# ssheybani/baby-vision-curriculum

Hardware: AMD Instinct MI355X
Metric: video clips/sec (node) VideoMAE-base 16x224^2 bf16 pretraining (higher is better)
Workload: dtype bf16; 1 GPU; VideoMAE-base (ViT-B/16 encoder, 4-layer decoder), 16x224x224 clips, tubelet 2, 90% tube mask, full training step (fwd + MSE + bwd + GradScaler + SGD-Nesterov); clips_per_gpu=256, global_batch=256, parallelism=dp1, weights=random init N(0,0.02), seed 0

## Files before the change

__graft_entry__.py:

```python
import importlib.util
import os
import subprocess
import sys

ROOT = os.path.dirname(os.path.abspath(__file__))
PKG_DIR = os.path.join(ROOT, "baby-vision-curriculum_amd")
CSRC = os.path.join(PKG_DIR, "csrc")
LIB = os.path.join(PKG_DIR, "libbvc_hip.so")
PRODUCT_SOURCES = ["gemm.hip", "gemm_persist.hip", "gemm8.hip", "gemm_as.hip", "attention.hip", "attention_probs.hip", "retrieval.hip", "separability.hip", "rowops.hip", "optim_layerwise.hip", "stack.hip", "context.hip", "ops.hip", "augment.hip", "randaug.hip", "jpeg.hip", "videomae.hip", "jepa.hip", "comm.hip"]
EXPERIMENT_SOURCES = [os.path.join("experiments", "gemm_big.hip"), os.path.join("experiments", "gemm_pp.hip")]
EXPERIMENT_INCLUDES = [os.path.join("experiments", "attention_dq_wave96.inc")]
HEADERS = ["common.h", "dropgate.h", "augment.h", "randaug.h", "jpeg.h", "gemm.h", "gemm_tile.h", "gemm_kernel_body.inc", "attention.h", "attention_fwd_body.inc", "attention_dq_body.inc", "attention_dkdv_body.inc", "rowops.h", "optim_layerwise.h", "stack.h", "context.h", os.path.join("..", "..", "include", "bvc.h")]


def _experiments():
    return "BVC_EXPERIMENTS" in os.environ.get("BVC_EXTRA_HIPCC_FLAGS", "")


def _sources():
    return PRODUCT_SOURCES + (EXPERIMENT_SOURCES if _experiments() else [])


SOURCES = PRODUCT_SOURCES


EXPERIMENT_FLAGS = {"attention.hip": ["-mllvm", "-amdgpu-mfma-vgpr-form=1"]}


def _extra_flags(src):
    return EXPERIMENT_FLAGS.get(src, []) if _experiments() else []


HASH_FILE = LIB + ".srchash"


def _source_hash():
    import hashlib
    h = hashlib.sha256()
    for f in _sources() + HEADERS + (EXPERIMENT_INCLUDES if _experiments() else []):
        with open(os.path.join(CSRC, f), "rb") as fh:
            h.update(f.encode() + b"\0" + fh.read())
    h.update(os.environ.get("BVC_EXTRA_HIPCC_FLAGS", "").encode())
    return h.hexdigest()


def _stale():
    if not (os.path.exists(LIB) and os.path.exists(HASH_FILE)):
        return True
    with open(HASH_FILE) as fh:
        return fh.read().strip() != _source_hash()


def _hash_of(files):
    import hashlib
    h = hashlib.sha256()
    for f in files:
        with open(os.path.join(CSRC, f), "rb") as fh:
            h.update(f.encode() + b"\0" + fh.read())
    return h.hexdigest()


def build(force: bool = False) -> None:
    if force or _stale():
        from concurrent.futures import ThreadPoolExecutor
        hipcc = os.environ.get("HIPCC", "/opt/rocm/bin/hipcc")
        objdir = os.path.join(PKG_DIR, "build")
        os.makedirs(objdir, exist_ok=True)
        flags = ["--offload-arch=gfx950", "-O3", "-std=c++17", "-fPIC"] + os.environ.get("BVC_EXTRA_HIPCC_FLAGS", "").split()

        def compile_one(src):
            obj = os.path.join(objdir, os.path.basename(src).replace(".hip", ".o"))
            stamp = obj + ".hash"
            fl = flags + _extra_flags(src) + ["-I" + CSRC]
            want = _hash_of([src] + HEADERS + (EXPERIMENT_INCLUDES if _experiments() else [])) + " " + " ".join(fl)
            if not force and os.path.exists(obj) and os.path.exists(stamp) and open(stamp).read() == want:
                return obj
            cmd = [hipcc, *fl, "-c", os.path.join(CSRC, src), "-o", obj]
            if src == "gemm8.hip":
                r = subprocess.run(cmd + ["-Rpass-analysis=kernel-resource-usage"], stderr=subprocess.PIPE, text=True)
                if r.returncode != 0:
                    sys.stderr.write(r.stderr)
                    raise subprocess.CalledProcessError(r.returncode, cmd)
                name = None
                for line in r.stderr.splitlines():
                    if "Function Name:" in line:
                        name = line.split("Function Name:")[1].split()[0]
                    elif "VGPRs Spill:" in line and name and "gemm8_kernel" in name and name.endswith("ELi0EEEvNS_9GemmGroupEi"):
                        if int(line.split("VGPRs Spill:")[1].split()[0]) != 0:
                            raise RuntimeError(f"gemm8.hip: {name} spills VGPRs; its counted-wait epilogue assumes none")
            else:
                subprocess.run(cmd, check=True)
            with open(stamp, "w") as fh:
# ... 59 lines not shown
```

baby-vision-curriculum_amd/csrc/gemm.h:

```cpp
#pragma once
#include "common.h"
#include "dropgate.h"
#include "../../include/bvc.h"

namespace bvc {

enum GemmLayout { GEMM_NT = BVC_GEMM_NT, GEMM_NN = BVC_GEMM_NN, GEMM_TN = BVC_GEMM_TN };

enum GemmEpilogue {
    EPI_F32 = BVC_EPI_F32,
    EPI_BF16 = BVC_EPI_BF16,
    EPI_GELU = BVC_EPI_GELU,
    EPI_RESID = BVC_EPI_RESID,
    EPI_POS = BVC_EPI_POS,
    EPI_E2D = BVC_EPI_E2D,
    EPI_LOSS = BVC_EPI_LOSS,
    EPI_DGELU = BVC_EPI_DGELU,
    EPI_F32_BF16 = BVC_EPI_F32_BF16,
    EPI_RELU = BVC_EPI_RELU,
    EPI_DRELU = BVC_EPI_DRELU,
    EPI_NCE = BVC_EPI_NCE,
    EPI_NCE_BWD = BVC_EPI_NCE_BWD,
    EPI_RESID_LN = BVC_EPI_RESID_LN,
    EPI_DLN = BVC_EPI_DLN,
    EPI_RESID_GATE = BVC_EPI_RESID_GATE
};

using GemmProblem = bvc_gemm_desc;

constexpr int kMaxGroup = 4;

struct Options { int gemm8 = 0; int dw_overlap = 0; int row_ln = 0; int row_stagger = 1; int deterministic = 0; int head_pad = 0; int dec_tail = 1; int dec_first = -1; };
Options& options();

float* det_scratch(size_t floats, hipStream_t stream);
size_t det_scratch_bytes();
int det_scratch_release();

struct DryRun { bool on = false; char name[160] = ""; };
DryRun& dry_run();

constexpr size_t operand_tail_bytes(size_t bf16_columns) { return 64 * bf16_columns * 2 + 1024; }
constexpr bool tn_tail_ok(int K, int ld) { return K % 64 == 0 || ((size_t)K + 63) / 64 * 64 * (size_t)ld * 2 + 1024 <= 0x100000000ull; }

int launch_gemm(const GemmProblem* probs, int nprob, GemmLayout layout, int tile_cfg, hipStream_t stream, int stages = -1);

int launch_gemm_gate(const GemmProblem& p, const Gate& gate, int tile_cfg, hipStream_t stream);

int gemm_num_tiles(const GemmProblem& p, int tile_cfg);
int gemm_pick_tile(const GemmProblem* probs, int nprob, int tile_cfg);
bool gemm_row_ln_ok(int M, int N, int K);
constexpr size_t kRowLnPartFloats = 512 * 2 * 384;

}
```

baby-vision-curriculum_amd/csrc/gemm.hip:

```cpp
#include <stdio.h>
#include <stdlib.h>
#include <string.h>

#include <algorithm>
#include <mutex>
#include <vector>

#include "gemm_tile.h"

namespace bvc {

Options& options() {
    static Options o;
    return o;
}
DryRun& dry_run() {
    static thread_local DryRun d;
    return d;
}

template <int BM, int BN, bool AT, bool BT, int NS, int LB = 2, bool EARLY_ = true>
__global__ __launch_bounds__(256, LB) void gemm_kernel(const GemmGroup g) {
    constexpr bool DET = false;
#include "gemm_kernel_body.inc"
// ... 46 lines not shown

namespace {
struct DetBuf { int dev; hipStream_t stream; float* ptr; size_t floats; };
std::mutex& det_mutex() { static std::mutex m; return m; }
std::vector<DetBuf>& det_bufs() { static std::vector<DetBuf> v; return v; }
}

float* det_scratch(size_t floats, hipStream_t stream) {
    int dev = 0;
    if (hipGetDevice(&dev) != hipSuccess) { set_error("det_scratch: hipGetDevice failed"); return nullptr; }
    std::lock_guard<std::mutex> lock(det_mutex());
    for (DetBuf& b : det_bufs()) {
        if (b.dev != dev || b.stream != stream) continue;
        if (b.floats >= floats) return b.ptr;
        if (hipStreamSynchronize(stream) != hipSuccess || hipFree(b.ptr) != hipSuccess) {
            set_error("det_scratch: releasing the old workspace failed");
            return nullptr;
        }
        const size_t want = std::max(floats, b.floats + b.floats / 2);
        b.ptr = nullptr; b.floats = 0;
        if (hipMalloc(&b.ptr, want * sizeof(float)) != hipSuccess) {
            set_error("det_scratch: hipMalloc of %zu bytes failed", want * sizeof(float));
            b.ptr = nullptr;
            return nullptr;
        }
        b.floats = want;
        return b.ptr;
    }
    DetBuf b{dev, stream, nullptr, floats};
    if (hipMalloc(&b.ptr, floats * sizeof(float)) != hipSuccess) {
        set_error("det_scratch: hipMalloc of %zu bytes failed", floats * sizeof(float));
        return nullptr;
    }
    det_bufs().push_back(b);
    return b.ptr;
}

int det_scratch_release() {
    int dev = 0;
    BVC_CHECK_HIP(hipGetDevice(&dev));
    std::lock_guard<std::mutex> lock(det_mutex());
    BVC_CHECK_HIP(hipDeviceSynchronize());
    std::vector<DetBuf>& v = det_bufs();
    for (size_t i = 0; i < v.size();) {
        if (v[i].dev != dev) { ++i; continue; }
        BVC_CHECK_HIP(hipFree(v[i].ptr));
        v.erase(v.begin() + i);
    }
    return BVC_OK;
}

size_t det_scratch_bytes() {
    int dev = 0;
    if (hipGetDevice(&dev) != hipSuccess) return 0;
    std::lock_guard<std::mutex> lock(det_mutex());
    size_t n = 0;
    for (const DetBuf& b : det_bufs())
        if (b.dev == dev) n += b.floats * sizeof(float);
    return n;
}

static void tile_dims(int cfg, int& bm, int& bn) {
    if (cfg == 10 || cfg == 11) { bm = 256; bn = cfg == 10 ? 256 : 128; return; }
    if (cfg == 12) { bm = 128; bn = 384; return; }
    if (cfg == 14) { bm = 128; bn = 256; return; }
    bm = cfg == 2 ? 64 : 128;
    bn = cfg == 0 ? 128 : 64;
}

static int tiles_for(const GemmProblem& p, int cfg) {
    int bm, bn;
    tile_dims(cfg, bm, bn);
    return ((p.M + bm - 1) / bm) * ((p.N + bn - 1) / bn);
}

bool gemm_row_ln_ok(int M, int N, int K) { return N == 384 && K % 64 == 0 && K >= 128 && M > 0 && (double)M * 1536.0 < 4294000000.0; }

int gemm_pick_tile(const GemmProblem* probs, int nprob, int tile_cfg) {
    if (tile_cfg == 6 || tile_cfg == 7) return tile_cfg - 6;
    if (tile_cfg == 9) return 0;
    if (tile_cfg >= 10 && tile_cfg <= 12) return tile_cfg;
    if (tile_cfg == 14) return tile_cfg;
    if (tile_cfg >= 15 && tile_cfg <= 18) return 0;
    if (tile_cfg >= 0) return tile_cfg;
    int t0 = 0, t1 = 0, nmax = 0;
    for (int i = 0; i < nprob; ++i) {
        t0 += tiles_for(probs[i], 0) * probs[i].split_k;
        t1 += tiles_for(probs[i], 1) * probs[i].split_k;
        nmax = probs[i].N > nmax ? probs[i].N : nmax;
    }
    if (nmax <= 384) return t0 >= 1024 ? 0 : (t1 >= 256 ? 1 : 2);
    if (t0 >= 400) return 0;
    if (t1 >= 400) return 1;
    return 2;
}

static int pick_panel(const GemmProblem& p, int cfg, GemmLayout layout) {
    if (BVC_EXP_ENV("BVC_GEMM_LEGACY_WALK") != nullptr) return 0;
    if (const char* pe = BVC_EXP_ENV("BVC_GEMM_PANEL")) {
        const int tn = (p.N + (cfg == 10 ? 256 : 128) - 1) / (cfg == 10 ? 256 : 128), gq = atoi(pe);
        if (layout != GEMM_TN && gq > 0) return gq < tn ? gq : tn;
    }
    if (layout == GEMM_TN) return 0;
    int bm, bn;
    tile_dims(cfg, bm, bn);
    const int tiles_m = (p.M + bm - 1) / bm, tiles_n = (p.N + bn - 1) / bn;
    const double kper = (double)((p.K + p.split_k - 1) / p.split_k);
    const double a_slab = bm * kper * 2.0, b_slab = bn * kper * 2.0, cap = 2.0 * 1024 * 1024;
    const double rows_x = tiles_m / 8.0 > 1.0 ? tiles_m / 8.0 : 1.0;
    auto cost = [&](int G) {
        const double npan = (double)((tiles_n + G - 1) / G);
        const double waves = rows_x * G / 64.0 > 1.0 ? rows_x * G / 64.0 : 1.0;
        return rows_x * a_slab * npan + tiles_n * b_slab * (G * b_slab <= cap ? 1.0 : waves);
    };
    int gmax = (int)(cap / b_slab);
    if ((cfg == 10 || cfg == 11) && gmax < 2) {
        const int gq = cfg == 10 ? 6 : 8;
        return gq < tiles_n ? gq : tiles_n;
    }
    if (gmax < 1) gmax = 1;
    if (gmax >= tiles_n) return tiles_n;
    const int npan = (tiles_n + gmax - 1) / gmax;
    const int G = (tiles_n + npan - 1) / npan;
    return cost(G) < cost(tiles_n) ? G : tiles_n;
}

static int pick_gemm8(const GemmProblem* probs, int nprob, GemmLayout layout);
int gemm_num_tiles(const GemmProblem& p, int tile_cfg) {
    if (tile_cfg < 0) {
        const int g8 = pick_gemm8(&p, 1, GEMM_NT);
        if (g8 > 0) tile_cfg = g8;
    }
    return tiles_for(p, gemm_pick_tile(&p, 1, tile_cfg));
}

template <int BM, int BN, bool AT, bool BT, int NS, int LB = 2, bool EARLY = true>
static int launch_one(const GemmGroup& g, int nblocks, hipStream_t stream) {
    constexpr size_t lds = (size_t)NS * (BM + BN) * 64 * 2;
    if (dry_run().on) {
        snprintf(dry_run().name, sizeof(dry_run().name), "bvc::gemm_kernel<%d, %d, %s, %s, %d, %d, %s>", BM, BN, AT ? "true" : "false",
                 BT ? "true" : "false", NS, LB, EARLY ? "true" : "false");
        return BVC_OK;
    }
    static bool attr_set = false;
    if (lds > 65536 && !attr_set) {
        BVC_CHECK_HIP(hipFuncSetAttribute(reinterpret_cast<const void*>(&gemm_kernel<BM, BN, AT, BT, NS, LB, EARLY>),
                                          hipFuncAttributeMaxDynamicSharedMemorySize, (int)lds));
        attr_set = true;
    }
    hipLaunchKernelGGL((gemm_kernel<BM, BN, AT, BT, NS, LB, EARLY>), dim3(nblocks), dim3(256), lds, stream, g);
    BVC_CHECK_HIP(hipGetLastError());
    return BVC_OK;
}

template <int BM, int BN, bool AT, bool BT>
static int launch_det_one(const GemmGroup& g, int nblocks, hipStream_t stream) {
    constexpr size_t lds = (size_t)2 * (BM + BN) * 64 * 2;
    static_assert(lds <= 65536, "gemm_det_kernel: dynamic LDS above 64 KiB would need the attribute");
    if (dry_run().on) {
        snprintf(dry_run().name, sizeof(dry_run().name), "bvc::gemm_det_kernel<%d, %d, %s, %s>", BM, BN, AT ? "true" : "false", BT ? "true" : "false");
        return BVC_OK;
    }
    hipLaunchKernelGGL((gemm_det_kernel<BM, BN, AT, BT>), dim3(nblocks), dim3(256), lds, stream, g);
    BVC_CHECK_HIP(hipGetLastError());
    return BVC_OK;
}

template <int BM, int BN>
static int launch_det_cfg(const GemmGroup& g, GemmLayout layout, int nblocks, hipStream_t stream) {
    switch (layout) {
        case GEMM_NT: return launch_det_one<BM, BN, false, false>(g, nblocks, stream);
        case GEMM_NN: return launch_det_one<BM, BN, false, true>(g, nblocks, stream);
        case GEMM_TN: return launch_det_one<BM, BN, true, true>(g, nblocks, stream);
        default: set_error("launch_gemm: bad layout %d", (int)layout); return BVC_ERR_INVALID;
    }
}

template <int BM, int BN, int NS>
static int launch_cfg(const GemmGroup& g, GemmLayout layout, int nblocks, hipStream_t stream) {
    switch (layout) {
        case GEMM_NT: return launch_one<BM, BN, false, false, NS>(g, nblocks, stream);
        case GEMM_NN: return launch_one<BM, BN, false, true, NS>(g, nblocks, stream);
        case GEMM_TN: return launch_one<BM, BN, true, true, NS>(g, nblocks, stream);
        default: set_error("launch_gemm: bad layout %d", (int)layout); return BVC_ERR_INVALID;
    }
}

template <int BM, int BN>
static int launch_stages(const GemmGroup& g, GemmLayout layout, int stages, int nblocks, hipStream_t stream) {
    if (stages == 3 && layout == GEMM_TN) return launch_one<BM, BN, true, true, 2, 1>(g, nblocks, stream);
    if (stages == 4) {
        if (layout == GEMM_NT) return launch_one<BM, BN, false, false, 2, 2, false>(g, nblocks, stream);
        if (layout == GEMM_NN) return launch_one<BM, BN, false, true, 2, 2, false>(g, nblocks, stream);
        return launch_one<BM, BN, true, true, 2, 2, false>(g, nblocks, stream);
    }
    return launch_cfg<BM, BN, 2>(g, layout, nblocks, stream);
}

int gemm_pick_stages(int, GemmLayout, int, int stages) { return (stages == 3 || stages == 4) ? stages : 2; }

int launch_gemm_big_nt(const GemmProblem& p, int cfg, hipStream_t stream);
int launch_gemm_persist(const GemmGroup& g, GemmLayout layout, int cfg, hipStream_t stream, int defer);
int launch_gemm8(const GemmGroup& g, GemmLayout layout, int bn, hipStream_t stream, bool det = false);
int launch_gemm_as(const GemmProblem& p, GemmLayout layout, int variant, hipStream_t stream);
bool gemm_as_ok(const GemmProblem& p, GemmLayout layout);
int launch_gemm_pp(const GemmGroup& g, GemmLayout layout, hipStream_t stream);

static int pick_gemm8(const GemmProblem* probs, int nprob, GemmLayout layout) {
    const int mode = options().gemm8;
    if (mode < 0 || nprob != 1 || layout == GEMM_TN) return -1;
    const GemmProblem& p = probs[0];
    if (p.split_k != 1 || p.K % 64 != 0) return -1;
    if (p.a_bytes >= 0x80000000u || p.b_bytes >= 0x80000000u) return -1;
    const bool gated = p.epi == EPI_DGELU || p.epi == EPI_DRELU;
    const bool bf = p.epi == EPI_BF16 || p.epi == EPI_GELU || p.epi == EPI_RELU;
    const bool resid = (p.epi == EPI_RESID || p.epi == EPI_POS || p.epi == EPI_F32 || p.epi == EPI_LOSS) && layout == GEMM_NT;
    if (!bf && !resid && !gated) return -1;
    const int tm = (p.M + 255) / 256, tn256 = (p.N + 255) / 256, tn128 = (p.N + 127) / 128;
    const bool fits256 = !bf || (size_t)tn256 * 256 * 4 <= 32768, fits128 = !bf || (size_t)tn128 * 128 * 4 <= 32768;
    if (mode > 0) {
        if (fits256 && (gated || p.N > 128)) return 10;
        return fits128 && !gated ? 11 : -1;
    }
    if (2.0 * p.M * p.N * p.K < 45e9) return -1;
    const bool full256 = (double)p.N >= 0.85 * 256.0 * tn256;
    if (full256 && fits256 && tm * tn256 >= 448) return 10;
    if (gated) return -1;
    if (p.epi != EPI_LOSS && fits128 && (bf ? layout == GEMM_NN : p.N <= 384) && p.K >= 1024 && tm * tn128 >= (resid ? 1024 : 224)) return 11;
    return -1;
}

template <int BM, int BN>
static int launch_gate_one(const GemmGroup& g, const Gate& gate, int nblocks, hipStream_t stream) {
    constexpr size_t lds = (size_t)2 * (BM + BN) * 64 * 2;
    static_assert(lds <= 65536, "gemm_gate_kernel: dynamic LDS above 64 KiB would need the attribute");
    if (dry_run().on) {
        snprintf(dry_run().name, sizeof(dry_run().name), "bvc::gemm_gate_kernel<%d, %d>", BM, BN);
        return BVC_OK;
    }
    hipLaunchKernelGGL((gemm_gate_kernel<BM, BN>), dim3(nblocks), dim3(256), lds, stream, g, gate);
    BVC_CHECK_HIP(hipGetLastError());
    return BVC_OK;
}

int launch_gemm_gate(const GemmProblem& p0, const Gate& gate, int tile_cfg, hipStream_t stream) {
    GemmProblem p = p0;
    p.epi = EPI_RESID_GATE;
    BVC_REQUIRE(tile_cfg >= -1 && tile_cfg <= 2, "launch_gemm_gate: tile config %d (the gated epilogue runs on tile configs 0 / 1 / 2)", tile_cfg);
    BVC_REQUIRE(p.M > 0 && p.N > 0 && p.K > 0, "launch_gemm_gate: empty problem (%d,%d,%d)", p.M, p.N, p.K);
    BVC_REQUIRE(p.N % 8 == 0 && p.K % 64 == 0, "launch_gemm_gate: N=%d must be a multiple of 8 and K=%d of 64", p.N, p.K);
    BVC_REQUIRE(p.lda % 8 == 0 && p.ldb % 8 == 0 && p.ldc % 8 == 0, "launch_gemm_gate: leading dims must be multiples of 8");
    BVC_REQUIRE(p.split_k == 1, "launch_gemm_gate: split_k must be 1");
    BVC_REQUIRE(p.A && p.B && p.C && p.resid, "launch_gemm_gate: null operand, output or residual");
    BVC_REQUIRE(gate.rows >= 1 && (double)p.M * p.N < 4398046511104.0, "launch_gemm_gate: bad gate (rows per sample %d) or more than 2^42 elements", gate.rows);
    const int cfg = gemm_pick_tile(&p, 1, tile_cfg);
    GemmGroup g;
    g.nprob = 1;
    g.bal_units = g.bal_lb = g.bal_tiles = 0;
    g.accum = 0;
    g.stagger = 0;
    g.dbg = 0;
    const int total = tiles_for(p, cfg);
    for (int i = 0; i < kMaxGroup; ++i) { g.prob[i] = p; g.panel[i] = pick_panel(p, cfg, GEMM_NT); g.tile_start[i] = i == 0 ? 0 : total; }
    g.tile_start[kMaxGroup] = total;
    switch (cfg) {
        case 0: return launch_gate_one<128, 128>(g, gate, total, stream);
        case 1: return launch_gate_one<128, 64>(g, gate, total, stream);
        default: return launch_gate_one<64, 64>(g, gate, total, stream);
    }
}

int launch_gemm(const GemmProblem* probs, int nprob, GemmLayout layout, int tile_cfg, hipStream_t stream, int stages) {
    BVC_REQUIRE(nprob >= 1 && nprob <= kMaxGroup, "launch_gemm: nprob %d out of range", nprob);
    for (int i = 0; i < nprob; ++i)
        BVC_REQUIRE(probs[i].epi != EPI_RESID_GATE, "launch_gemm: BVC_EPI_RESID_GATE needs its gate (bvc_op_gemm_gate / a context with bvc_*_set_drop)");
    static thread_local bool skip_g8 = false;
    bool auto_g8 = false;
    if (probs[0].epi == EPI_RESID_LN || probs[0].epi == EPI_DLN) {
        const GemmProblem& p = probs[0];
        BVC_REQUIRE(nprob == 1 && (tile_cfg < 0 || tile_cfg == 12), "launch_gemm: the LayerNorm epilogues take one problem on tile config 12");
        BVC_REQUIRE(gemm_row_ln_ok(p.M, p.N, p.K) && p.ldc == p.N && p.split_k == 1 && p.a_bytes < 0x80000000u && p.b_bytes < 0x80000000u,
                    "launch_gemm: the LayerNorm epilogues need N == ldc == 384, K %% 64 == 0, operands below 2 GiB (M=%d N=%d K=%d)", p.M, p.N, p.K);
        BVC_REQUIRE(p.C && p.C2 && p.ln_mean && p.ln_rstd && p.ln_gamma, "launch_gemm: LayerNorm epilogue with a null output / statistic / scale");
        if (p.epi == EPI_RESID_LN) BVC_REQUIRE(layout == GEMM_NT && p.resid && p.ln_beta, "launch_gemm: RESID_LN is an NT product with a residual and a LayerNorm bias");
        if (p.epi == EPI_DLN) BVC_REQUIRE(layout == GEMM_NN && p.ln_x && p.ln_part && p.ln_dgamma && p.ln_dbeta, "launch_gemm: DLN is an NN product with the LayerNorm input, partial scratch and parameter gradients");
        if (p.seg_rows != 0)
            BVC_REQUIRE(p.seg_rows > 0 && p.seg_rows % 128 == 0 && p.M % p.seg_rows == 0 && p.seg_off >= 0 && p.seg_stride > 0 &&
                            (long long)p.seg_off + p.seg_rows <= (long long)p.seg_stride,
                        "launch_gemm: bad segment map (seg_rows %d: a multiple of 128 that divides M = %d; seg_off %d + seg_rows <= seg_stride %d)",
                        p.seg_rows, p.M, p.seg_off, p.seg_stride);
        tile_cfg = 12;
    } else {
        for (int i = 0; i < nprob; ++i)
            BVC_REQUIRE(probs[i].seg_rows == 0, "launch_gemm: a segment map (seg_rows %d) exists for BVC_EPI_RESID_LN / BVC_EPI_DLN only", probs[i].seg_rows);
    }
    if (tile_cfg < 0 && stages < 0 && nprob == 1 && options().gemm8 >= 0 && probs[0].epi == EPI_BF16 && gemm_as_ok(probs[0], layout) &&
        (options().gemm8 > 0 || probs[0].M >= 16384) && BVC_EXP_ENV("BVC_GEMM_NO_AS") == nullptr)
        return launch_gemm_as(probs[0], layout, 0, stream);
    if (tile_cfg < 0 && stages < 0 && !skip_g8) {
        const int g8 = pick_gemm8(probs, nprob, layout);
        if (g8 > 0) { tile_cfg = g8; auto_g8 = true; }
    }
    if (tile_cfg >= 15 && tile_cfg <= 18) {
        BVC_REQUIRE(nprob == 1, "launch_gemm: tile configs 15 - 18 take one problem");
        const int rc = launch_gemm_as(probs[0], layout, tile_cfg - 15, stream);
        BVC_REQUIRE(rc != 1, "launch_gemm: tile configs 15 - 18 (A-stationary kernel) take NT products with K = 384, N %% 128 == 0, BF16 / GELU epilogues");
        return rc;
    }
    if ((tile_cfg >= 3 && tile_cfg <= 5) || tile_cfg == 8) {
#ifdef BVC_EXPERIMENTS
        BVC_REQUIRE(nprob == 1 && layout == GEMM_NT, "launch_gemm: tile configs 3-5 (32-deep K steps) are NT, one problem");
        BVC_REQUIRE(!options().deterministic || probs[0].split_k == 1, "launch_gemm: tile configs 3-5 have no deterministic split-K form");
        return launch_gemm_big_nt(probs[0], tile_cfg, stream);
#else
        BVC_REQUIRE(false, "launch_gemm: tile configs 3-5 / 8 exist only in a -DBVC_EXPERIMENTS build (csrc/experiments/gemm_big.hip)");
#endif
    }
    bool accum = false;
    if (tile_cfg == 13) {
        BVC_REQUIRE(layout == GEMM_TN, "launch_gemm: tile config 13 (accumulating 256 x 256 tiles) is for weight gradients (TN)");
        for (int i = 0; i < nprob; ++i) BVC_REQUIRE(probs[i].epi == EPI_F32, "launch_gemm: tile config 13 takes plain f32 outputs");
        accum = true;
        tile_cfg = 10;
    }
    const int cfg = gemm_pick_tile(probs, nprob, tile_cfg);
    GemmGroup g;
    g.nprob = nprob;
    g.bal_units = g.bal_lb = g.bal_tiles = 0;
    g.accum = accum ? 1 : 0;
    g.stagger = 0;
    {
        const char* e = BVC_EXP_ENV("BVC_GEMM_DEBUG");
        g.dbg = e ? atoi(e) : 0;
    }
    int total = 0;
    for (int i = 0; i < nprob; ++i) {
        const GemmProblem& p = probs[i];
        BVC_REQUIRE(p.M > 0 && p.N > 0 && p.K > 0, "launch_gemm: empty problem %d (%d,%d,%d)", i, p.M, p.N, p.K);
        BVC_REQUIRE(p.N % 8 == 0, "launch_gemm: N=%d must be a multiple of 8", p.N);
        BVC_REQUIRE(p.lda % 8 == 0 && p.ldb % 8 == 0 && p.ldc % 8 == 0, "launch_gemm: leading dims must be multiples of 8");
        if (layout != GEMM_TN) BVC_REQUIRE(p.K % 64 == 0, "launch_gemm: K=%d must be a multiple of 64 for k-contiguous operands", p.K);
        if (layout == GEMM_TN) BVC_REQUIRE(p.M % 8 == 0, "launch_gemm: TN needs M %% 8 == 0 (M=%d)", p.M);
        if (layout == GEMM_TN)
            BVC_REQUIRE(tn_tail_ok(p.K, p.lda) && tn_tail_ok(p.K, p.ldb),
                        "launch_gemm: TN with K=%d (no multiple of 64), lda=%d, ldb=%d: the 32-bit byte offsets of the rows past K in the last K step "
                        "would wrap past 4 GiB into the operand instead of reading as zero", p.K, p.lda, p.ldb);
        BVC_REQUIRE(p.split_k >= 1, "launch_gemm: split_k must be >= 1");
        if (p.rowsum) BVC_REQUIRE(layout == GEMM_TN, "launch_gemm: rowsum (bias gradient) is fused into TN products only");
        if (p.split_k > 1)
            BVC_REQUIRE(p.epi == EPI_F32 || (p.epi == EPI_RESID && p.resid == p.C),
                        "launch_gemm: split_k needs an accumulating f32 epilogue");
        g.prob[i] = p;
        g.panel[i] = pick_panel(p, cfg, layout);
        if (cfg >= 10 && cfg <= 12 && layout == GEMM_TN && BVC_EXP_ENV("BVC_G8_TN_LEGACY_WALK") == nullptr) {
            int bm, bn;
            tile_dims(cfg, bm, bn);
            g.panel[i] = (p.N + bn - 1) / bn;
            if (BVC_EXP_ENV("BVC_G8_TN_SHORT_FAST") != nullptr) g.panel[i] = -1;
        }
        g.tile_start[i] = total;
        total += tiles_for(p, cfg) * p.split_k;
    }
    g.tile_start[nprob] = total;
    for (int i = nprob; i < kMaxGroup; ++i) { g.prob[i] = probs[0]; g.panel[i] = g.panel[0]; g.tile_start[i + 1] = total; }
    if (options().deterministic) {
        DetReduce r;
        memset(&r, 0, sizeof(r));
        r.nprob = nprob;
        size_t floats = 0;
        long long items = 0;
        size_t at[kMaxGroup][2];
        for (int i = 0; i < nprob; ++i) {
            const GemmProblem& p = probs[i];
            const bool slab = p.split_k > 1 || accum;
            r.start[i] = items;
            r.M[i] = p.M; r.N[i] = p.N; r.ldc[i] = p.ldc; r.S[i] = p.split_k;
            at[i][0] = at[i][1] = (size_t)-1;
// ... 88 lines not shown
```

baby-vision-curriculum_amd/csrc/ops.hip:

```cpp
#include <stdarg.h>
#include <stdio.h>
#include <string.h>

#include "context.h"
#include "optim_layerwise.h"

namespace bvc {
static thread_local char g_err[1024] = "";
void set_error(const char* fmt, ...) {
    va_list ap;
    va_start(ap, fmt);
    vsnprintf(g_err, sizeof(g_err), fmt, ap);
    va_end(ap);
}
const char* last_error() { return g_err; }
}

using namespace bvc;

extern "C" {

const char* bvc_last_error(void) { return bvc::last_error(); }
const char* bvc_version(void) { return "gfx950;bvc-hip-r5"; }

int bvc_set_option(const char* name, int value) {
    BVC_REQUIRE(name != nullptr, "set_option: null name");
    if (!strcmp(name, "gemm8")) { BVC_REQUIRE(value >= -1 && value <= 1, "set_option: gemm8 takes -1 / 0 / 1"); options().gemm8 = value; }
    else if (!strcmp(name, "dw_overlap")) options().dw_overlap = value != 0;
    else if (!strcmp(name, "row_stagger")) options().row_stagger = value != 0;
    else if (!strcmp(name, "row_ln")) { BVC_REQUIRE(value >= -1 && value <= 1, "set_option: row_ln takes -1 / 0 / 1"); options().row_ln = value; }
    else if (!strcmp(name, "deterministic")) { BVC_REQUIRE(value == 0 || value == 1, "set_option: deterministic takes 0 / 1"); options().deterministic = value; }
    else if (!strcmp(name, "head_pad")) { BVC_REQUIRE(value == 0 || value == 1, "set_option: head_pad takes 0 / 1"); options().head_pad = value; }
    else if (!strcmp(name, "dec_tail")) { BVC_REQUIRE(value == 0 || value == 1, "set_option: dec_tail takes 0 / 1"); options().dec_tail = value; }
    else if (!strcmp(name, "dec_first")) { BVC_REQUIRE(value >= -1 && value <= 1, "set_option: dec_first takes -1 / 0 / 1"); options().dec_first = value; }
    else BVC_REQUIRE(false, "set_option: unknown option '%s'", name);
    return BVC_OK;
}
int bvc_get_option(const char* name) {
    if (name && !strcmp(name, "gemm8")) return options().gemm8;
    if (name && !strcmp(name, "dw_overlap")) return options().dw_overlap;
    if (name && !strcmp(name, "row_ln")) return options().row_ln;
    if (name && !strcmp(name, "row_stagger")) return options().row_stagger;
    if (name && !strcmp(name, "deterministic")) return options().deterministic;
    if (name && !strcmp(name, "head_pad")) return options().head_pad;
    if (name && !strcmp(name, "dec_tail")) return options().dec_tail;
    if (name && !strcmp(name, "dec_first")) return options().dec_first;
    bvc::set_error("get_option: unknown option '%s'", name ? name : "(null)");
    return BVC_ERR_INVALID;
}

int bvc_op_gemm(const bvc_gemm_desc* problems, int count, int layout, int tile_cfg, int stages, void* stream) {
    BVC_REQUIRE(problems, "op_gemm: null problems");
    BVC_REQUIRE(layout >= 0 && layout <= 2, "op_gemm: bad layout %d", layout);
    return launch_gemm(problems, count, (GemmLayout)layout, tile_cfg, (hipStream_t)stream, stages);
}
static int op_gate(const bvc_branch_drop* drop, int layer, int branch, int M, Gate* g) {
    BVC_REQUIRE(drop && layer >= 0 && layer < (1 << 22) && (branch == 0 || branch == 1), "gate: null description, or layer / branch out of range");
    BVC_REQUIRE(drop->hidden_p >= 0.f && drop->hidden_p < 1.f && drop->rows_per_sample >= 1, "gate: hidden_p outside [0, 1) or rows_per_sample < 1");
    const int samples = (M + drop->rows_per_sample - 1) / drop->rows_per_sample;
    *g = make_gate(drop->hidden_p, drop->seed, drop->offset,
                   drop->path_scale ? drop->path_scale + ((size_t)layer * 2 + branch) * samples : nullptr, drop->rows_per_sample, layer, branch);
    return BVC_OK;
}
int bvc_op_gemm_gate(const bvc_gemm_desc* problem, const bvc_branch_drop* drop, int layer, int branch, int tile_cfg, void* stream) {
    BVC_REQUIRE(problem, "op_gemm_gate: null problem");
    Gate g;
    TRY(op_gate(drop, layer, branch, problem->M, &g));
    return launch_gemm_gate(*problem, g, tile_cfg, (hipStream_t)stream);
}
int bvc_op_gemm_gate_kernel(const bvc_gemm_desc* problem, int tile_cfg, char* name, int name_cap) {
    BVC_REQUIRE(problem && name && name_cap > 0, "op_gemm_gate_kernel: null argument");
    DryRun& d = dry_run();
    d.on = true;
    d.name[0] = 0;
    const int rc = launch_gemm_gate(*problem, make_gate(0.f, 0, 0, nullptr, 1, 0, 0), tile_cfg, nullptr);
    d.on = false;
    if (rc == BVC_OK) snprintf(name, name_cap, "%s", d.name);
    return rc;
}
int bvc_op_dropout_mask(uint64_t seed, uint64_t offset, int layer, int branch, int M, int N, float p, uint8_t* out_dev, void* stream) {
    BVC_REQUIRE(out_dev && M >= 1 && N >= 1 && layer >= 0 && layer < (1 << 22) && (branch == 0 || branch == 1) && p >= 0.f && p < 1.f,
                "op_dropout_mask: bad argument");
    return launch_dropout_mask(make_gate(p, seed, offset, nullptr, 1, layer, branch), (size_t)M * N, out_dev, (hipStream_t)stream);
}
int bvc_dropout_mask_host(uint64_t seed, uint64_t offset, int layer, int branch, int M, int N, float p, uint8_t* out_host) {
    BVC_REQUIRE(out_host && M >= 1 && N >= 1 && layer >= 0 && layer < (1 << 22) && (branch == 0 || branch == 1) && p >= 0.f && p < 1.f,
                "dropout_mask_host: bad argument");
    dropout_mask_host(make_gate(p, seed, offset, nullptr, 1, layer, branch), (size_t)M * N, out_host);
    return BVC_OK;
}
int bvc_op_layernorm_bwd_gate(const void* dy, const float* x, const float* mean, const float* rstd, const float* gamma, float* dres,
                              int accumulate, void* dres_bf16, float* dgamma, float* dbeta, float* workspace, int M, int D,
                              const bvc_branch_drop* drop, int layer, int branch, void* stream) {
    Gate g;
    TRY(op_gate(drop, layer, branch, M, &g));
    return launch_ln_bwd((const bf16_t*)dy, x, identity_rows(), mean, rstd, gamma, dres, accumulate, (bf16_t*)dres_bf16, dgamma, dbeta,
                         workspace, M, D, (hipStream_t)stream, &g);
}
int bvc_op_gemm_kernel(const bvc_gemm_desc* problems, int count, int layout, int tile_cfg, int stages, char* name, int name_cap) {
    BVC_REQUIRE(problems && name && name_cap > 0, "op_gemm_kernel: null argument");
    BVC_REQUIRE(layout >= 0 && layout <= 2, "op_gemm_kernel: bad layout %d", layout);
    DryRun& d = dry_run();
    d.on = true;
    d.name[0] = 0;
    const int rc = launch_gemm(problems, count, (GemmLayout)layout, tile_cfg, nullptr, stages);
    d.on = false;
    if (rc == BVC_OK) snprintf(name, name_cap, "%s", d.name);
    return rc;
}
int64_t bvc_deterministic_workspace_bytes(void) { return (int64_t)det_scratch_bytes(); }
int bvc_deterministic_workspace_release(void) { return det_scratch_release(); }
int bvc_op_gemm_plan_dw(bvc_gemm_desc* problems, int count) {
    BVC_REQUIRE(problems && count >= 1 && count <= 4, "op_gemm_plan_dw: bad argument");
    return plan_dw(problems, count);
}
int bvc_op_gemm_num_tiles(const bvc_gemm_desc* problem, int tile_cfg) {
    if (!problem) return BVC_ERR_INVALID;
    return gemm_num_tiles(*problem, tile_cfg);
}
int bvc_op_attention_fwd(const void* qkv, void* ctx_out, float* lse, int B, int N, int H, int head_dim, void* stream) {
    BVC_REQUIRE(qkv && ctx_out && lse, "op_attention_fwd: null argument");
    return launch_attn_fwd((const bf16_t*)qkv, (bf16_t*)ctx_out, lse, B, N, H, head_dim, (hipStream_t)stream);
}
int bvc_op_attention_bwd(const void* qkv, const void* ctx_in, const void* dctx, const float* lse, float* delta, void* dqkv,
                         int B, int N, int H, int head_dim, void* stream) {
    BVC_REQUIRE(qkv && ctx_in && dctx && lse && delta && dqkv, "op_attention_bwd: null argument");
    return launch_attn_bwd((const bf16_t*)qkv, (const bf16_t*)ctx_in, (const bf16_t*)dctx, lse, delta, (bf16_t*)dqkv, B, N, H, head_dim,
                           (hipStream_t)stream);
}
// ... 248 lines not shown
```

Baseline: 3256 clips/s.

## Add weight-stationary persistent GEMM kernel for K=384 products

Adds a persistent GEMM kernel for K=384 products that keeps a 192-column slice of the weight matrix in registers for the whole launch. It streams 128-row A tiles through a six-slot LDS ring using counted vmcnt waits, and fuses bias, GELU or dGELU epilogues. With default options it is used for large-M BF16 NT and DGELU NN products, which fit the decoder or MLP shapes. The aim is to avoid re-loading B per tile and to hide A-load latency, at the cost of one block per CU and high register pressure.

```diff
diff --git a/__graft_entry__.py b/__graft_entry__.py
--- a/__graft_entry__.py
+++ b/__graft_entry__.py
@@ -7,7 +7,7 @@
 PKG_DIR = os.path.join(ROOT, "baby-vision-curriculum_amd")
 CSRC = os.path.join(PKG_DIR, "csrc")
 LIB = os.path.join(PKG_DIR, "libbvc_hip.so")
-PRODUCT_SOURCES = ["gemm.hip", "gemm_persist.hip", "gemm8.hip", "gemm_as.hip", "attention.hip", "attention_probs.hip", "retrieval.hip", "separability.hip", "rowops.hip", "optim_layerwise.hip", "stack.hip", "context.hip", "ops.hip", "augment.hip", "randaug.hip", "jpeg.hip", "videomae.hip", "jepa.hip", "comm.hip"]
+PRODUCT_SOURCES = ["gemm.hip", "gemm_persist.hip", "gemm8.hip", "gemm_as.hip", "gemm_ws.hip", "attention.hip", "attention_probs.hip", "retrieval.hip", "separability.hip", "rowops.hip", "optim_layerwise.hip", "stack.hip", "context.hip", "ops.hip", "augment.hip", "randaug.hip", "jpeg.hip", "videomae.hip", "jepa.hip", "comm.hip"]
 EXPERIMENT_SOURCES = [os.path.join("experiments", "gemm_big.hip"), os.path.join("experiments", "gemm_pp.hip")]
 EXPERIMENT_INCLUDES = [os.path.join("experiments", "attention_dq_wave96.inc")]
 HEADERS = ["common.h", "dropgate.h", "augment.h", "randaug.h", "jpeg.h", "gemm.h", "gemm_tile.h", "gemm_kernel_body.inc", "attention.h", "attention_fwd_body.inc", "attention_dq_body.inc", "attention_dkdv_body.inc", "rowops.h", "optim_layerwise.h", "stack.h", "context.h", os.path.join("..", "..", "include", "bvc.h")]
diff --git a/baby-vision-curriculum_amd/csrc/gemm.h b/baby-vision-curriculum_amd/csrc/gemm.h
--- a/baby-vision-curriculum_amd/csrc/gemm.h
+++ b/baby-vision-curriculum_amd/csrc/gemm.h
@@ -30,7 +30,7 @@
 
 constexpr int kMaxGroup = 4;
 
-struct Options { int gemm8 = 0; int dw_overlap = 0; int row_ln = 0; int row_stagger = 1; int deterministic = 0; int head_pad = 0; int dec_tail = 1; int dec_first = -1; };
+struct Options { int gemm8 = 0; int dw_overlap = 0; int row_ln = 0; int row_stagger = 1; int deterministic = 0; int head_pad = 0; int dec_tail = 1; int dec_first = -1; int gemm_ws = 0; };
 Options& options();
 
 float* det_scratch(size_t floats, hipStream_t stream);
diff --git a/baby-vision-curriculum_amd/csrc/gemm.hip b/baby-vision-curriculum_amd/csrc/gemm.hip
--- a/baby-vision-curriculum_amd/csrc/gemm.hip
+++ b/baby-vision-curriculum_amd/csrc/gemm.hip
@@ -152,6 +152,7 @@
     if (tile_cfg >= 10 && tile_cfg <= 12) return tile_cfg;
     if (tile_cfg == 14) return tile_cfg;
     if (tile_cfg >= 15 && tile_cfg <= 18) return 0;
+    if (tile_cfg == 19) return 0;
     if (tile_cfg >= 0) return tile_cfg;
     int t0 = 0, t1 = 0, nmax = 0;
     for (int i = 0; i < nprob; ++i) {
@@ -274,6 +275,8 @@
 int launch_gemm8(const GemmGroup& g, GemmLayout layout, int bn, hipStream_t stream, bool det = false);
 int launch_gemm_as(const GemmProblem& p, GemmLayout layout, int variant, hipStream_t stream);
 bool gemm_as_ok(const GemmProblem& p, GemmLayout layout);
+int launch_gemm_ws(const GemmProblem& p, GemmLayout layout, hipStream_t stream);
+bool gemm_ws_ok(const GemmProblem& p, GemmLayout layout);
 int launch_gemm_pp(const GemmGroup& g, GemmLayout layout, hipStream_t stream);
 
 static int pick_gemm8(const GemmProblem* probs, int nprob, GemmLayout layout) {
@@ -298,6 +301,12 @@
     if (gated) return -1;
     if (p.epi != EPI_LOSS && fits128 && (bf ? layout == GEMM_NN : p.N <= 384) && p.K >= 1024 && tm * tn128 >= (resid ? 1024 : 224)) return 11;
     return -1;
+}
+
+static bool ws_selected(const GemmProblem& p, GemmLayout layout) {
+    if (p.M < 131072 || p.N < 1152) return false;
+    if (p.epi == EPI_DGELU) return layout == GEMM_NN;
+    return p.epi == EPI_BF16 && layout == GEMM_NT && p.M < 262144;
 }
 
 template <int BM, int BN>
@@ -363,6 +372,15 @@
     } else {
         for (int i = 0; i < nprob; ++i)
             BVC_REQUIRE(probs[i].seg_rows == 0, "launch_gemm: a segment map (seg_rows %d) exists for BVC_EPI_RESID_LN / BVC_EPI_DLN only", probs[i].seg_rows);
+    }
+    if (tile_cfg < 0 && stages < 0 && nprob == 1 && options().gemm_ws >= 0 && gemm_ws_ok(probs[0], layout) &&
+        (options().gemm_ws > 0 || ws_selected(probs[0], layout)))
+        return launch_gemm_ws(probs[0], layout, stream);
+    if (tile_cfg == 19) {
+        BVC_REQUIRE(nprob == 1, "launch_gemm: tile config 19 takes one problem");
+        const int rc = launch_gemm_ws(probs[0], layout, stream);
+        BVC_REQUIRE(rc != 1, "launch_gemm: tile config 19 (weight-stationary kernel) takes NT / NN products with K = 384, N %% 192 == 0, BF16 / GELU / DGELU epilogues");
+        return rc;
     }
     if (tile_cfg < 0 && stages < 0 && nprob == 1 && options().gemm8 >= 0 && probs[0].epi == EPI_BF16 && gemm_as_ok(probs[0], layout) &&
         (options().gemm8 > 0 || probs[0].M >= 16384) && BVC_EXP_ENV("BVC_GEMM_NO_AS") == nullptr)
diff --git a/baby-vision-curriculum_amd/csrc/gemm_ws.hip b/baby-vision-curriculum_amd/csrc/gemm_ws.hip
--- /dev/null
+++ b/baby-vision-curriculum_amd/csrc/gemm_ws.hip
@@ -0,0 +1,291 @@
+#include <stdio.h>
+#include <stdlib.h>
+
+#include <type_traits>
+
+#include "gemm_tile.h"
+
+namespace bvc {
+
+namespace {
+
+typedef __attribute__((ext_vector_type(4))) unsigned int u32x4;
+typedef __attribute__((ext_vector_type(2))) unsigned int u32x2;
+
+constexpr uint32_t kInvalidBase = 0x80000000u;
+constexpr uint32_t kDrop = 0xFFFFFFF0u;
+
+constexpr int WS_NKT = 6;
+constexpr int WS_SLICE = 192;
+constexpr int WS_SLOT = 128 * 64 * 2;
+constexpr int WS_RING = 6;
+constexpr int WS_DIST = 5;
+constexpr int WS_BIMG = WS_SLICE * 64 * 2;
+constexpr int WS_AUX_OFF = WS_RING * WS_SLOT;
+constexpr int WS_AUX_WAVE = 6 * 1024;
+constexpr int WS_BIAS_OFF = WS_AUX_OFF + 8 * WS_AUX_WAVE;
+constexpr size_t WS_LDS_BYTES = (size_t)WS_BIAS_OFF + WS_SLICE * 4;
+
+enum { WS_BF16 = 0, WS_GELU = 1, WS_DGELU = 2 };
+
+template <int E>
+constexpr int ws_extra(int kt) { return kt == 5 ? (E == WS_GELU ? 12 : 6) : (E == WS_DGELU && kt < 3 ? 2 : 0); }
+template <int E>
+constexpr int ws_cnt(int kt) {
+    int n = 2 * (WS_DIST - 1);
+    for (int d = 0; d < WS_DIST; ++d) n += ws_extra<E>((kt - d + WS_NKT) % WS_NKT);
+    return n;
+}
+
+}
+
+template <int E, bool BT>
+__global__ __launch_bounds__(512, 1) void gemm_ws_kernel(const GemmProblem p, const int nunits, const int nslices, const int pp) {
+    extern __shared__ __attribute__((aligned(16))) char smem[];
+    static_assert(WS_LDS_BYTES <= 160 * 1024, "LDS per CU");
+    static_assert(WS_DIST <= WS_RING - 1 && 3 * WS_BIMG <= WS_BIAS_OFF, "ring: a slot is re-staged one barrier after its last read");
+    static_assert(ws_cnt<WS_GELU>(5) <= 63 && WS_DIST == WS_NKT - 1, "vmcnt is a 6-bit counter; the prologue stands for steps 1 - 5");
+
+    const int tid = threadIdx.x, lane = tid & 63;
+    const int wave = __builtin_amdgcn_readfirstlane(tid >> 6);
+    const int wm = wave >> 2, wn = wave & 3;
+    const int q4 = lane >> 4, r16 = lane & 15;
+    const int lda = p.lda, ldb = p.ldb, ldc = p.ldc, Mrows = p.M;
+    const float alpha = p.alpha_dev ? p.alpha * p.alpha_dev[0] : p.alpha;
+
+    const int xcd = blockIdx.x & 7, local = blockIdx.x >> 3;
+    const int pl = local / nslices, slice = local - pl * nslices;
+    int uid = pl * 8 + xcd;
+    const int ustep = 8 * pp;
+    if (pl >= pp || uid >= nunits) return;
+    const int n0 = slice * WS_SLICE;
+
+    const __amdgpu_buffer_rsrc_t ra = make_rsrc(p.A, p.a_bytes), rb = make_rsrc(p.B, p.b_bytes);
+    const uint32_t lds0 = (uint32_t)(size_t)((AS3 char*)smem);
+    const uint32_t lds_w = lds0 + (uint32_t)wave * 1024u;
+    const int r8 = 8 * wave + (lane >> 3);
+
+    {
+        AS3 float* lb_ = (AS3 float*)((AS3 char*)smem + WS_BIAS_OFF);
+        for (int i = tid; i < WS_SLICE; i += 512) lb_[i] = p.bias ? p.bias[n0 + i] : 0.f;
+    }
+
+    bf16x8 bfr[3][2 * WS_NKT];
+    {
+        uint32_t lb;
+        if constexpr (!BT) lb = (uint32_t)(((n0 + r8) * ldb + (((lane & 7) ^ swz_rows(r8)) << 3)) * 2);
+        else lb = (uint32_t)((r8 * ldb + n0 + (((lane & 7) ^ swz_tr<64>(r8)) << 3)) * 2);
+#pragma unroll
+        for (int half = 0; half < 2; ++half) {
+#pragma unroll
+            for (int ktl = 0; ktl < 3; ++ktl) {
+                const int kt = 3 * half + ktl;
+#pragma unroll
+                for (int jj = 0; jj < 3; ++jj) {
+                    const uint32_t off = BT ? (uint32_t)((64 * kt * ldb + 64 * jj) * 2) : (uint32_t)((64 * jj * ldb + 64 * kt) * 2);
+                    glds16(rb, lb + off, lds_w + (uint32_t)(ktl * WS_BIMG + jj * 8192));
+                }
+            }
+            wait_vmcnt<0>();
+            __syncthreads();
+#pragma unroll
+            for (int ktl = 0; ktl < 3; ++ktl)
+#pragma unroll
+                for (int ks = 0; ks < 2; ++ks)
+#pragma unroll
+                    for (int j = 0; j < 3; ++j) {
+                        const char* img = smem + ktl * WS_BIMG;
+                        if constexpr (!BT) {
+                            bfr[j][2 * (3 * half + ktl) + ks] = read_frag<128, false>(img, 48 * wn + 16 * j, ks, lane);
+                        } else {
+                            const int ct = 3 * wn + j;
+                            bfr[j][2 * (3 * half + ktl) + ks] = read_frag<64, true>(img + (ct >> 2) * 8192, (ct & 3) * 16, ks, lane);
+                        }
+                    }
+            asm volatile("s_waitcnt lgkmcnt(0)" ::: "memory");
+            __syncthreads();
+        }
+    }
+
+    const uint32_t la = (uint32_t)((r8 * lda + (((lane & 7) ^ swz_rows(r8)) << 3)) * 2);
+    int s_uid = uid, s_kt = 0, s_slot = 0;
+    auto stage = [&]() {
+        const uint32_t dst = lds_w + (uint32_t)(s_slot * WS_SLOT);
+        const uint32_t base = s_uid < nunits ? (uint32_t)s_uid * 128u * (uint32_t)lda * 2u + (uint32_t)(s_kt * 128) : kInvalidBase;
+        glds16(ra, la + base, dst);
+        glds16(ra, la + base + (uint32_t)(64 * lda * 2), dst + 8192u);
+        if (++s_slot == WS_RING) s_slot = 0;
+        if (++s_kt == WS_NKT) { s_kt = 0; s_uid += ustep; }
+    };
+    const AS3 float* lbias = (const AS3 float*)((AS3 char*)smem + WS_BIAS_OFF);
+    const uint32_t cext = (uint32_t)Mrows * (uint32_t)ldc * 2u;
+    const __amdgpu_buffer_rsrc_t rc = make_rsrc(p.C, cext), rc2 = make_rsrc(E == WS_GELU ? p.C2 : p.C, cext);
+    const int ldx = E == WS_DGELU ? p.ldaux : 0;
+    const __amdgpu_buffer_rsrc_t rx = make_rsrc(E == WS_DGELU ? p.aux : p.A, (uint32_t)Mrows * (uint32_t)ldx * 2u);
+    const uint32_t lds_x = lds0 + (uint32_t)(WS_AUX_OFF + wave * WS_AUX_WAVE);
+    const AS3 char* aux_w = (const AS3 char*)smem + WS_AUX_OFF + wave * WS_AUX_WAVE;
+
+#pragma unroll
+    for (int i = 0; i < WS_DIST; ++i) {
+        stage();
+#pragma unroll
+        for (int s = 0; s < ws_extra<E>(i + 1); ++s) glds16(ra, (uint32_t)lane * 16u, lds_x + (uint32_t)((s % 6) * 1024));
+    }
+    wait_vmcnt<ws_cnt<E>(WS_NKT - 1)>();
+    asm volatile("s_barrier" ::: "memory");
+
+    auto pair_lane = [&](int i, int ld) {
+        const int row = 64 * wm + (i < 4 ? 0 : 16 * (q4 & 1)) + r16, col = n0 + 48 * wn + (i < 4 ? 16 * (q4 & 1) : 32) + 8 * (q4 >> 1);
+        return (uint32_t)((row * ld + col) * 2);
+    };
+    auto pair_unit = [&](int i, int m0, int ld) {
+        uint32_t s = (uint32_t)(m0 + (i < 4 ? 16 * i : 32 * (i - 4))) * (uint32_t)ld * 2u;
+        asm volatile("" : "+s"(s));
+        return s;
+    };
+    const uint32_t coA = pair_lane(0, ldc), coB = pair_lane(4, ldc), xoA = pair_lane(0, ldx), xoB = pair_lane(4, ldx);
+
+    int r_slot = 0;
+    f32x4 acc[4][3];
+    bf16x8 afr[4][2];
+    while (true) {
+        const int m0 = uid * 128;
+#pragma unroll
+        for (int i = 0; i < 4; ++i)
+#pragma unroll
+            for (int j = 0; j < 3; ++j) acc[i][j] = f32x4{0.f, 0.f, 0.f, 0.f};
+
+        auto epi_pair = [&](auto i_) {
+            constexpr int i = decltype(i_)::value;
+            constexpr int rtX = i < 4 ? i : 2 * (i - 4), jX = i < 4 ? 0 : 2, rtY = i < 4 ? i : 2 * (i - 4) + 1, jY = i < 4 ? 1 : 2;
+            const f32x4 bX = *reinterpret_cast<const AS3 f32x4*>(lbias + 48 * wn + 16 * jX + 4 * q4);
+            const f32x4 bY = *reinterpret_cast<const AS3 f32x4*>(lbias + 48 * wn + 16 * jY + 4 * q4);
+            float va[4], vb[4], ga[4], gb[4];
+#pragma unroll
+            for (int e = 0; e < 4; ++e) {
+                va[e] = acc[rtX][jX][e] * alpha + bX[e];
+                vb[e] = acc[rtY][jY][e] * alpha + bY[e];
+            }
+            if constexpr (E == WS_GELU) { gelu_split(va, ga); gelu_split(vb, gb); }
+            if constexpr (E == WS_DGELU) {
+                const AS3 char* ax = aux_w + i * 1024 + ((q4 >> 1) * 32 + r16) * 16 + (q4 & 1) * 8;
+                const u32x2 wX = *reinterpret_cast<const AS3 u32x2*>(ax), wY = *reinterpret_cast<const AS3 u32x2*>(ax + 256);
+#pragma unroll
+                for (int e = 0; e < 2; ++e) {
+                    va[2 * e] *= __uint_as_float(wX[e] << 16);
+                    va[2 * e + 1] *= __uint_as_float(wX[e] & 0xffff0000u);
+                    vb[2 * e] *= __uint_as_float(wY[e] << 16);
+                    vb[2 * e + 1] *= __uint_as_float(wY[e] & 0xffff0000u);
+                }
+            }
+            const uint32_t o = (i < 4 ? coA : coB) + pair_unit(i, m0, ldc);
+            auto emit = [&](__amdgpu_buffer_rsrc_t r, const float (&x)[4], const float (&y)[4]) {
+                const uint32_t a0 = pack2bf(x[0], x[1]), a1 = pack2bf(x[2], x[3]);
+                const uint32_t c0 = pack2bf(y[0], y[1]), c1 = pack2bf(y[2], y[3]);
+                const auto s0 = __builtin_amdgcn_permlane16_swap(a0, c0, false, false);
+                const auto s1 = __builtin_amdgcn_permlane16_swap(a1, c1, false, false);
+                __builtin_amdgcn_raw_buffer_store_b128(u32x4{s0[0], s1[0], s0[1], s1[1]}, r, o, 0, 0);
+            };
+            emit(rc, va, vb);
+            if constexpr (E == WS_GELU) emit(rc2, ga, gb);
+        };
+
+        auto kstep = [&](auto kt_) {
+            constexpr int kt = decltype(kt_)::value;
+            __builtin_amdgcn_sched_barrier(0);
+            const char* slot = smem + r_slot * WS_SLOT;
+#pragma unroll
+            for (int ks = 0; ks < 2; ++ks)
+#pragma unroll
+                for (int rt = 0; rt < 4; ++rt) afr[rt][ks] = read_frag<128, false>(slot, 64 * wm + 16 * rt, ks, lane);
+            stage();
+            if constexpr (E == WS_DGELU && kt < 3) {
+#pragma unroll
+                for (int i = 2 * kt; i < 2 * kt + 2; ++i) {
+                    glds16(rx, (i < 4 ? xoA : xoB) + pair_unit(i, m0, ldx), lds_x + (uint32_t)(i * 1024));
+                }
+            }
+            __builtin_amdgcn_s_setprio(1);
+#pragma unroll
+            for (int ks = 0; ks < 2; ++ks)
+#pragma unroll
+                for (int rt = 0; rt < 4; ++rt)
+#pragma unroll
+                    for (int j = 0; j < 3; ++j)
+                        acc[rt][j] = __builtin_amdgcn_mfma_f32_16x16x32_bf16(bfr[j][2 * kt + ks], afr[rt][ks], acc[rt][j], 0, 0, 0);
+            __builtin_amdgcn_s_setprio(0);
+            if constexpr (kt == WS_NKT - 1) {
+                __builtin_amdgcn_sched_barrier(0);
+                if constexpr (E == WS_DGELU) wait_vmcnt<2 * 3>();
+                epi_pair(std::integral_constant<int, 0>{}); epi_pair(std::integral_constant<int, 1>{});
+                epi_pair(std::integral_constant<int, 2>{}); epi_pair(std::integral_constant<int, 3>{});
+                epi_pair(std::integral_constant<int, 4>{}); epi_pair(std::integral_constant<int, 5>{});
+            }
+            __builtin_amdgcn_sched_barrier(0);
+            wait_vmcnt<ws_cnt<E>(kt)>();
+            asm volatile("s_waitcnt lgkmcnt(0)\n\ts_barrier" ::: "memory");
+            if (++r_slot == WS_RING) r_slot = 0;
+        };
+        kstep(std::integral_constant<int, 0>{}); kstep(std::integral_constant<int, 1>{}); kstep(std::integral_constant<int, 2>{});
+        kstep(std::integral_constant<int, 3>{}); kstep(std::integral_constant<int, 4>{}); kstep(std::integral_constant<int, 5>{});
+        uid += ustep;
+        if (uid >= nunits) break;
+    }
+    wait_vmcnt<0>();
+}
+
+static int ws_ncu() {
+    static int ncu = 0;
+    if (ncu == 0) {
+        int dev = 0;
+        hipDeviceProp_t prop;
+        if (hipGetDevice(&dev) != hipSuccess || hipGetDeviceProperties(&prop, dev) != hipSuccess) return 256;
+        ncu = prop.multiProcessorCount > 0 ? prop.multiProcessorCount : 256;
+    }
+    return ncu;
+}
+
+bool gemm_ws_ok(const GemmProblem& p, GemmLayout layout) {
+    if ((layout != GEMM_NT && layout != GEMM_NN) || p.K != 384 || p.N <= 0 || p.N % WS_SLICE != 0 || p.N / WS_SLICE > 32 || p.split_k != 1) return false;
+    if (p.epi != EPI_BF16 && p.epi != EPI_GELU && p.epi != EPI_DGELU) return false;
+    if (p.epi == EPI_GELU && p.C2 == nullptr) return false;
+    if (p.epi == EPI_DGELU && (p.aux == nullptr || p.ldaux % 8 != 0 || p.ldaux < p.N || ((size_t)p.M + 256) * p.ldaux * 2 >= kInvalidBase)) return false;
+    if (p.a_bytes >= kInvalidBase || p.b_bytes >= kInvalidBase || ((size_t)p.M + 256) * p.ldc * 2 >= 0xFFFFFFF0ull) return false;
+    if (((size_t)p.M + 256) * p.lda * 2 >= 0xFFFFFFF0ull) return false;
+    if (p.seg_rows != 0) return false;
+    return p.lda % 8 == 0 && p.ldb % 8 == 0 && p.ldc % 8 == 0 && p.M > 0;
+}
+
+template <int E, bool BT>
+static int launch_ws_one(const GemmProblem& p, hipStream_t stream) {
+    if (dry_run().on) {
+        snprintf(dry_run().name, sizeof(dry_run().name), "bvc::gemm_ws_kernel<%d, %s>", E, BT ? "true" : "false");
+        return BVC_OK;
+    }
+    static bool attr_set = false;
+    if (!attr_set) {
+        BVC_CHECK_HIP(hipFuncSetAttribute(reinterpret_cast<const void*>(&gemm_ws_kernel<E, BT>), hipFuncAttributeMaxDynamicSharedMemorySize,
+                                          (int)WS_LDS_BYTES));
+        attr_set = true;
+    }
+    const int nunits = (p.M + 127) / 128, nslices = p.N / WS_SLICE;
+    int per_xcd = ws_ncu() / 8;
+    if (per_xcd < nslices) per_xcd = nslices;
+    int pp = per_xcd / nslices;
+    if (pp > (nunits + 7) / 8) pp = (nunits + 7) / 8;
+    hipLaunchKernelGGL((gemm_ws_kernel<E, BT>), dim3(8 * pp * nslices), dim3(512), WS_LDS_BYTES, stream, p, nunits, nslices, pp);
+    BVC_CHECK_HIP(hipGetLastError());
+    return BVC_OK;
+}
+
+int launch_gemm_ws(const GemmProblem& p, GemmLayout layout, hipStream_t stream) {
+    if (!gemm_ws_ok(p, layout)) return 1;
+    const bool bt = layout == GEMM_NN;
+    switch (p.epi) {
+        case EPI_BF16: return bt ? launch_ws_one<WS_BF16, true>(p, stream) : launch_ws_one<WS_BF16, false>(p, stream);
+        case EPI_GELU: return bt ? launch_ws_one<WS_GELU, true>(p, stream) : launch_ws_one<WS_GELU, false>(p, stream);
+        default: return bt ? launch_ws_one<WS_DGELU, true>(p, stream) : launch_ws_one<WS_DGELU, false>(p, stream);
+    }
+}
+
+}
diff --git a/baby-vision-curriculum_amd/csrc/ops.hip b/baby-vision-curriculum_amd/csrc/ops.hip
--- a/baby-vision-curriculum_amd/csrc/ops.hip
+++ b/baby-vision-curriculum_amd/csrc/ops.hip
@@ -33,6 +33,7 @@
     else if (!strcmp(name, "head_pad")) { BVC_REQUIRE(value == 0 || value == 1, "set_option: head_pad takes 0 / 1"); options().head_pad = value; }
     else if (!strcmp(name, "dec_tail")) { BVC_REQUIRE(value == 0 || value == 1, "set_option: dec_tail takes 0 / 1"); options().dec_tail = value; }
     else if (!strcmp(name, "dec_first")) { BVC_REQUIRE(value >= -1 && value <= 1, "set_option: dec_first takes -1 / 0 / 1"); options().dec_first = value; }
+    else if (!strcmp(name, "gemm_ws")) { BVC_REQUIRE(value >= -1 && value <= 1, "set_option: gemm_ws takes -1 / 0 / 1"); options().gemm_ws = value; }
     else BVC_REQUIRE(false, "set_option: unknown option '%s'", name);
     return BVC_OK;
 }
@@ -45,6 +46,7 @@
     if (name && !strcmp(name, "head_pad")) return options().head_pad;
     if (name && !strcmp(name, "dec_tail")) return options().dec_tail;
     if (name && !strcmp(name, "dec_first")) return options().dec_first;
+    if (name && !strcmp(name, "gemm_ws")) return options().gemm_ws;
     bvc::set_error("get_option: unknown option '%s'", name ? name : "(null)");
     return BVC_ERR_INVALID;
 }
```

Result: no change. 3276 clips/s (median of 6 runs) (+0.6%).
